# jiwoon-ahn/irn

Measured on AMD Instinct MI355X. Metric: images/sec for CAM+random-walk label gen, VOC12 512^2 (random-walk label generation stage), higher is better.
Workload: dtype f32

## Files before the change

irn_amd/csrc/label.hip:

```cpp
#include "kernels.hpp"

#pragma clang fp contract(off)

namespace irn {

struct LabelJob {
    const float *rw;
    const int64_t *keys;
    uint8_t *labels;
    int32_t *argmax;
    float *rw_up;
    unsigned *max_slot;
    int c, h, w, oh, ow;
    const uint8_t *gt;
};

namespace {

__device__ __forceinline__ unsigned enc_ordered(float f) {
    const unsigned b = __float_as_uint(f);
    return (b & 0x80000000u) ? ~b : (b | 0x80000000u);
}
__device__ __forceinline__ float dec_ordered(unsigned u) {
    return __uint_as_float((u & 0x80000000u) ? (u & 0x7fffffffu) : ~u);
}

struct Taps {
    int i0, i1;
    float l0, l1;
};

__device__ __forceinline__ Taps taps_x4(int dst, int n_in) {
    float src = ((float)dst + 0.5f) * 0.25f;
    src = src - 0.5f;
    src = src < 0.f ? 0.f : src;
    Taps t;
    t.i0 = min((int)src, n_in - 1);
    t.i1 = min(t.i0 + 1, n_in - 1);
    t.l1 = src - (float)t.i0;
    t.l0 = 1.0f - t.l1;
    return t;
}

__device__ __forceinline__ float bilerp(const float *__restrict__ plane, int w, const Taps &ty, const Taps &tx) {
    const float v00 = plane[ty.i0 * w + tx.i0], v01 = plane[ty.i0 * w + tx.i1];
    const float v10 = plane[ty.i1 * w + tx.i0], v11 = plane[ty.i1 * w + tx.i1];
    const float p01 = v01 * tx.l1, p11 = v11 * tx.l1;
    const float top = __builtin_fmaf(v00, tx.l0, p01);
    const float bot = __builtin_fmaf(v10, tx.l0, p11);
    const float pb = ty.l1 * bot;
    return __builtin_fmaf(ty.l0, top, pb);
}

__device__ __forceinline__ int cell_lo(int k) { return k == 0 ? 0 : 4 * k + 2; }

template <int PASS>
__global__ __launch_bounds__(256) void upsample_max_kernel(const LabelJob *__restrict__ jobs) {
    const LabelJob J = jobs[blockIdx.y];
    const unsigned plane_px = (unsigned)(J.h * J.w), cells = (unsigned)J.c * plane_px;
    const float lower = PASS == 2 ? dec_ordered(*J.max_slot) : 0.f;
    float m = -INFINITY;
    for (unsigned i = blockIdx.x * 256 + threadIdx.x; i < cells; i += gridDim.x * 256) {
        const int c = (int)(i / plane_px);
        const int r = (int)(i - (unsigned)c * plane_px);
        const int k = (int)((unsigned)r / (unsigned)J.w), l = r - k * J.w;
        const int y0 = cell_lo(k), x0 = cell_lo(l);
        if (y0 >= J.oh || x0 >= J.ow) continue;
        const float *plane = J.rw + (long)c * J.h * J.w;
        if (PASS == 1) {
            m = fmaxf(m, bilerp(plane, J.w, taps_x4(y0, J.h), taps_x4(x0, J.w)));
        } else {
            const int k1 = min(k + 1, J.h - 1), l1 = min(l + 1, J.w - 1);
            const float u = fmaxf(fmaxf(plane[k * J.w + l], plane[k * J.w + l1]), fmaxf(plane[k1 * J.w + l], plane[k1 * J.w + l1]));
            if (u + fabsf(u) * 1e-6f + 1e-37f < lower) continue;
            const int y1 = min(k == J.h - 1 ? 4 * J.h - 1 : 4 * k + 5, J.oh - 1);
            const int x1 = min(l == J.w - 1 ? 4 * J.w - 1 : 4 * l + 5, J.ow - 1);
            for (int oy = y0; oy <= y1; ++oy) {
                const Taps ty = taps_x4(oy, J.h);
                for (int ox = x0; ox <= x1; ++ox) m = fmaxf(m, bilerp(plane, J.w, ty, taps_x4(ox, J.w)));
            }
        }
    }
    for (int s = 32; s > 0; s >>= 1) m = fmaxf(m, __shfl_xor(m, s));
    __shared__ float wmax[4];
    if ((threadIdx.x & 63) == 0) wmax[threadIdx.x >> 6] = m;
    __syncthreads();
    if (threadIdx.x == 0) {
        m = fmaxf(fmaxf(wmax[0], wmax[1]), fmaxf(wmax[2], wmax[3]));
        if (m > -INFINITY) atomicMax(J.max_slot, enc_ordered(m));
    }
}

__device__ __forceinline__ float bilerp_vals(float v00, float v01, float v10, float v11, const Taps &ty, const Taps &tx) {
    const float p01 = v01 * tx.l1, p11 = v11 * tx.l1;
    const float top = __builtin_fmaf(v00, tx.l0, p01);
    const float bot = __builtin_fmaf(v10, tx.l0, p11);
    const float pb = ty.l1 * bot;
    return __builtin_fmaf(ty.l0, top, pb);
}

__global__ __launch_bounds__(256) void label_argmax_kernel(const LabelJob *__restrict__ jobs, float bg) {
    const LabelJob J = jobs[blockIdx.y];
    const unsigned gw = (unsigned)(J.ow + 3) >> 2, groups = gw * (unsigned)J.oh;
    const unsigned npx = (unsigned)J.oh * (unsigned)J.ow;
    const float gmax = dec_ordered(*J.max_slot);
    for (unsigned g = blockIdx.x * 256 + threadIdx.x; g < groups; g += gridDim.x * 256) {
        const int oy = (int)(g / gw), ox = (int)(g - (unsigned)oy * gw) * 4;
        const int nq = min(4, J.ow - ox);
        const Taps ty = taps_x4(oy, J.h);
        Taps tx[4];
#pragma unroll
        for (int q = 0; q < 4; ++q) tx[q] = taps_x4(min(ox + q, J.ow - 1), J.w);
        float best[4] = {bg, bg, bg, bg};
        int idx[4] = {0, 0, 0, 0};
        const unsigned o = (unsigned)oy * (unsigned)J.ow + (unsigned)ox;
        for (int c = 0; c < J.c; ++c) {
            const float *r0 = J.rw + (long)c * J.h * J.w + ty.i0 * J.w, *r1 = J.rw + (long)c * J.h * J.w + ty.i1 * J.w;
            const float a00 = r0[tx[0].i0], a01 = r0[tx[0].i1], a10 = r1[tx[0].i0], a11 = r1[tx[0].i1];
            const float b00 = r0[tx[2].i0], b01 = r0[tx[2].i1], b10 = r1[tx[2].i0], b11 = r1[tx[2].i1];
            float v[4];
            v[0] = bilerp_vals(a00, a01, a10, a11, ty, tx[0]) / gmax;
            v[1] = bilerp_vals(a00, a01, a10, a11, ty, tx[1]) / gmax;
            v[2] = bilerp_vals(b00, b01, b10, b11, ty, tx[2]) / gmax;
            v[3] = bilerp_vals(b00, b01, b10, b11, ty, tx[3]) / gmax;
            if (J.rw_up) {
                float *dst = J.rw_up + (long)c * npx + o;
                if (nq == 4 && ((uintptr_t)dst & 15) == 0) *reinterpret_cast<float4 *>(dst) = make_float4(v[0], v[1], v[2], v[3]);
                else
                    for (int q = 0; q < nq; ++q) dst[q] = v[q];
            }
#pragma unroll
            for (int q = 0; q < 4; ++q)
                if (v[q] > best[q] || (v[q] != v[q] && best[q] == best[q])) {
                    best[q] = v[q];
                    idx[q] = c + 1;
                }
        }
        if (J.argmax) {
            int32_t *dst = J.argmax + o;
            if (nq == 4 && ((uintptr_t)dst & 15) == 0) *reinterpret_cast<int4 *>(dst) = make_int4(idx[0], idx[1], idx[2], idx[3]);
            else
                for (int q = 0; q < nq; ++q) dst[q] = idx[q];
        }
        if (J.labels) {
            uint8_t lab[4];
#pragma unroll
            for (int q = 0; q < 4; ++q) lab[q] = idx[q] == 0 ? (uint8_t)0 : (uint8_t)(J.keys[idx[q] - 1] + 1);
            uint8_t *dst = J.labels + o;
            if (nq == 4 && ((uintptr_t)dst & 3) == 0)
                *reinterpret_cast<uint32_t *>(dst) = (uint32_t)lab[0] | ((uint32_t)lab[1] << 8) | ((uint32_t)lab[2] << 16) | ((uint32_t)lab[3] << 24);
            else
                for (int q = 0; q < nq; ++q) dst[q] = lab[q];
        }
    }
}

constexpr int kSweepGroups = 4;
constexpr int kSweepChunk = 256 * kSweepGroups;
constexpr int kSweepCap = 15360;
constexpr int kSweepRows = IRN_EVAL_CLASSES + 1;
constexpr int kSweepMaxC = IRN_EVAL_CLASSES - 1;
constexpr uint32_t kSweepSkip = 0xffffffffu;

__global__ __launch_bounds__(256) void label_sweep_kernel(const LabelJob *__restrict__ jobs, const float *__restrict__ thres,
                                                          int t, int cap, int64_t *__restrict__ hist, int64_t *__restrict__ bad) {
    extern __shared__ __attribute__((aligned(16))) uint32_t sweep_lds[];
    uint32_t *bins = sweep_lds;
    float *th = reinterpret_cast<float *>(sweep_lds + cap);
    int *col = reinterpret_cast<int *>(th + IRN_EVAL_MAX_THRES);
    uint32_t *nbad = reinterpret_cast<uint32_t *>(col + kSweepMaxC);
    const LabelJob J = jobs[blockIdx.y];
    const int tid = threadIdx.x;
    if (tid == 0) *nbad = 0;
    for (int i = tid; i < t; i += 256) th[i] = thres[i];
    if (tid < J.c) {
        const int64_t key = J.keys[tid];
        col[tid] = (key >= 0 && key < kSweepMaxC) ? (int)key + 1 : -1;
    }
    __syncthreads();
    uint32_t local_bad = 0;
    if (blockIdx.x == 0 && blockIdx.y == 0)
        for (int i = tid; i < t; i += 256)
            if (th[i] != th[i] || (i > 0 && !(th[i - 1] <= th[i]))) ++local_bad;

    const unsigned gw = (unsigned)(J.ow + 3) >> 2, groups = gw * (unsigned)J.oh;
    const unsigned chunks = (groups + kSweepChunk - 1) / kSweepChunk;
    const uint32_t nbins = (uint32_t)(t + 1) * kSweepRows * (uint32_t)J.c;
    const float gmax = dec_ordered(*J.max_slot);
    for (unsigned chunk = blockIdx.x; chunk < chunks; chunk += gridDim.x) {
        uint32_t bin[4 * kSweepGroups];
#pragma unroll
        for (int i = 0; i < kSweepGroups; ++i) {
#pragma unroll
            for (int q = 0; q < 4; ++q) bin[4 * i + q] = kSweepSkip;
            const unsigned g = chunk * kSweepChunk + (unsigned)i * 256 + (unsigned)tid;
            if (g >= groups) continue;
            const int oy = (int)(g / gw), ox = (int)(g - (unsigned)oy * gw) * 4;
            const int nq = min(4, J.ow - ox);
            const Taps ty = taps_x4(oy, J.h);
            Taps tx[4];
#pragma unroll
            for (int q = 0; q < 4; ++q) tx[q] = taps_x4(min(ox + q, J.ow - 1), J.w);
            float m[4] = {0.f, 0.f, 0.f, 0.f};
            int cs[4] = {0, 0, 0, 0}, nanc[4] = {-1, -1, -1, -1};
            for (int c = 0; c < J.c; ++c) {
                const float *r0 = J.rw + (long)c * J.h * J.w + ty.i0 * J.w, *r1 = J.rw + (long)c * J.h * J.w + ty.i1 * J.w;
                const float a00 = r0[tx[0].i0], a01 = r0[tx[0].i1], a10 = r1[tx[0].i0], a11 = r1[tx[0].i1];
                const float b00 = r0[tx[2].i0], b01 = r0[tx[2].i1], b10 = r1[tx[2].i0], b11 = r1[tx[2].i1];
                float v[4];
                v[0] = bilerp_vals(a00, a01, a10, a11, ty, tx[0]) / gmax;
                v[1] = bilerp_vals(a00, a01, a10, a11, ty, tx[1]) / gmax;
                v[2] = bilerp_vals(b00, b01, b10, b11, ty, tx[2]) / gmax;
                v[3] = bilerp_vals(b00, b01, b10, b11, ty, tx[3]) / gmax;
#pragma unroll
                for (int q = 0; q < 4; ++q) {
                    if (c == 0 || v[q] > m[q]) {
                        m[q] = v[q];
                        cs[q] = c;
                    }
                    if (v[q] != v[q] && nanc[q] < 0) nanc[q] = c;
                }
            }
            const uint8_t *gp = J.gt + ((unsigned)oy * (unsigned)J.ow + (unsigned)ox);
            uint8_t gv[4] = {0, 0, 0, 0};
            if (nq == 4 && ((uintptr_t)gp & 3) == 0) {
                const uint32_t u = *reinterpret_cast<const uint32_t *>(gp);
                gv[0] = (uint8_t)u; gv[1] = (uint8_t)(u >> 8); gv[2] = (uint8_t)(u >> 16); gv[3] = (uint8_t)(u >> 24);
            } else {
                for (int q = 0; q < nq; ++q) gv[q] = gp[q];
            }
#pragma unroll
            for (int q = 0; q < 4; ++q) {
                if (q >= nq) continue;
                const int row = gv[q] <= 20 ? (int)gv[q] : (gv[q] == 255 ? IRN_EVAL_CLASSES : -1);
                if (row < 0) {
                    ++local_bad;
                    continue;
                }
                int lo = 0, hi = t;
                while (lo < hi) {
                    const int mid = (lo + hi) >> 1;
                    if (th[mid] < m[q]) lo = mid + 1;
                    else hi = mid;
                }
                const int j = nanc[q] >= 0 ? t : lo, cq = nanc[q] >= 0 ? nanc[q] : cs[q];
                bin[4 * i + q] = ((uint32_t)j * kSweepRows + (uint32_t)row) * (uint32_t)J.c + (uint32_t)cq;
            }
        }
        for (uint32_t b0 = 0; b0 < nbins; b0 += (uint32_t)cap) {
            const uint32_t nb = min((uint32_t)cap, nbins - b0);
            for (uint32_t b = tid; b < nb; b += 256) bins[b] = 0;
            __syncthreads();
#pragma unroll
            for (int i = 0; i < 4 * kSweepGroups; ++i)
                if (bin[i] - b0 < nb) atomicAdd(&bins[bin[i] - b0], 1u);
            __syncthreads();
            for (uint32_t b = tid; b < nb; b += 256) {
                const uint32_t v = bins[b];
                if (!v) continue;
                const uint32_t id = b0 + b;
                const int c = (int)(id % (uint32_t)J.c);
                const uint32_t r = id / (uint32_t)J.c;
                const int row = (int)(r % kSweepRows), j = (int)(r / kSweepRows);
                if (col[c] < 0) {
                    local_bad += v;
                    continue;
                }
                atomicAdd(reinterpret_cast<unsigned long long *>(hist + ((size_t)row * IRN_EVAL_CLASSES + col[c]) * (t + 1) + j),
                          (unsigned long long)v);
            }
            __syncthreads();
        }
    }
    if (local_bad) atomicAdd(nbad, local_bad);
    __syncthreads();
    if (tid == 0 && *nbad) atomicAdd(reinterpret_cast<unsigned long long *>(bad), (unsigned long long)*nbad);
}

constexpr int kMaxScales = 8;
struct MergeArgs {
    const float *src[kMaxScales];
    int hs[kMaxScales], ws[kMaxScales];
    int n_scales, n_cls, k;
    const int64_t *keys;
    float *lo, *hi;
    int lh, lw, uh, uw, H, W;
    unsigned *max_slots;
};

__device__ __forceinline__ Taps taps_resize(int dst, int n_in, int n_out) {
    const float scale = (float)n_in / (float)n_out;
    float src = scale * ((float)dst + 0.5f);
    src = src - 0.5f;
    src = src < 0.f ? 0.f : src;
    Taps t;
    t.i0 = min((int)src, n_in - 1);
    t.i1 = min(t.i0 + 1, n_in - 1);
    t.l1 = src - (float)t.i0;
    t.l0 = 1.0f - t.l1;
    return t;
}

__global__ __launch_bounds__(256) void cam_merge_sum_kernel(const MergeArgs A) {
    const int kk = blockIdx.y;
    const bool is_hi = blockIdx.z == 1;
    const int oh = is_hi ? A.H : A.lh, ow = is_hi ? A.W : A.lw;
    const int th = is_hi ? A.uh : A.lh, tw = is_hi ? A.uw : A.lw;
    float *out = (is_hi ? A.hi : A.lo) + (long)kk * oh * ow;
    const int cls = (int)A.keys[kk];
    float m = -INFINITY;
    for (long o = (long)blockIdx.x * 256 + threadIdx.x; o < (long)oh * ow; o += (long)gridDim.x * 256) {
        const int oy = (int)(o / ow), ox = (int)(o - (long)oy * ow);
        float acc = 0.f;
        for (int s = 0; s < A.n_scales; ++s) {
            const Taps ty = taps_resize(oy, A.hs[s], th), tx = taps_resize(ox, A.ws[s], tw);
            acc = acc + bilerp(A.src[s] + (long)cls * A.hs[s] * A.ws[s], A.ws[s], ty, tx);
        }
        out[o] = acc;
        m = fmaxf(m, acc);
    }
    for (int s = 32; s > 0; s >>= 1) m = fmaxf(m, __shfl_xor(m, s));
    __shared__ float wmax[4];
    if ((threadIdx.x & 63) == 0) wmax[threadIdx.x >> 6] = m;
    __syncthreads();
    if (threadIdx.x == 0) {
        m = fmaxf(fmaxf(wmax[0], wmax[1]), fmaxf(wmax[2], wmax[3]));
        if (m > -INFINITY) atomicMax(A.max_slots + (is_hi ? A.k : 0) + kk, enc_ordered(m));
    }
}

__global__ __launch_bounds__(256) void cam_merge_norm_kernel(const MergeArgs A) {
    const int kk = blockIdx.y;
    const bool is_hi = blockIdx.z == 1;
    const long n = is_hi ? (long)A.H * A.W : (long)A.lh * A.lw;
    float *out = (is_hi ? A.hi : A.lo) + (long)kk * n;
    const float den = dec_ordered(A.max_slots[(is_hi ? A.k : 0) + kk]) + 1e-5f;
    for (long o = (long)blockIdx.x * 256 + threadIdx.x; o < n; o += (long)gridDim.x * 256) out[o] = out[o] / den;
}

}
}

using namespace irn;

extern "C" int irn_label_epilogue(int n_images, const float *const *rw_dev, const int32_t *c, const int32_t *h,
                                  const int32_t *w, const int32_t *out_h, const int32_t *out_w, float bg_thres,
                                  const int64_t *const *keys_dev, uint8_t *const *labels_dev,
                                  int32_t *const *argmax_dev, float *const *rw_up_dev, void *scratch_dev,
                                  void *stream_) {
    hipStream_t stream = (hipStream_t)stream_;
    if (n_images < 1 || !rw_dev || !c || !h || !w || !out_h || !out_w || !scratch_dev)
        return fail(IRN_ERR_ARG, "irn_label_epilogue: bad argument");
    std::vector<LabelJob> jobs(n_images);
    long max_px = 0, max_cells = 0;
    for (int i = 0; i < n_images; ++i) {
        LabelJob &J = jobs[i];
        if (!rw_dev[i] || c[i] < 1 || h[i] < 1 || w[i] < 1 || out_h[i] < 1 || out_w[i] < 1 ||
            out_h[i] > 4 * h[i] || out_w[i] > 4 * w[i])
            return fail(IRN_ERR_ARG, "irn_label_epilogue: image %d: bad sizes (c=%d %dx%d -> %dx%d)", i, c[i], h[i],
                        w[i], out_h[i], out_w[i]);
        J.rw = rw_dev[i];
        J.keys = keys_dev ? keys_dev[i] : nullptr;
        J.labels = labels_dev ? labels_dev[i] : nullptr;
        J.argmax = argmax_dev ? argmax_dev[i] : nullptr;
        J.rw_up = rw_up_dev ? rw_up_dev[i] : nullptr;
        if (J.labels && !J.keys)
            return fail(IRN_ERR_ARG, "irn_label_epilogue: image %d: labels requested without keys", i);
        J.max_slot = (unsigned *)scratch_dev + i;
        J.c = c[i]; J.h = h[i]; J.w = w[i]; J.oh = out_h[i]; J.ow = out_w[i];
        max_px = std::max(max_px, (long)out_h[i] * out_w[i]);
        max_cells = std::max(max_cells, (long)c[i] * h[i] * w[i]);
    }
    LabelJob *jobs_dev = nullptr;
    int rc = scratch_upload(jobs.data(), sizeof(LabelJob) * n_images, (void **)&jobs_dev, stream);
    if (rc) return rc;
    IRN_HIP_TRY(hipMemsetAsync(scratch_dev, 0, sizeof(unsigned) * n_images, stream));
    if (max_px >= (1L << 31) || max_cells >= (1L << 31)) return fail(IRN_ERR_ARG, "irn_label_epilogue: image too large (32-bit pixel indices)");
    const long per_image = std::max<long>(1, 4096 / n_images);
    const int bx = (int)std::min<long>((max_px / 4 + 255) / 256 + 1, 512);
    const int bc = (int)std::min<long>((max_cells + 255) / 256, per_image);
    hipLaunchKernelGGL(upsample_max_kernel<1>, dim3(bc, n_images), dim3(256), 0, stream, jobs_dev);
    IRN_LAUNCH_CHECK("upsample_max_kernel<1>");
    hipLaunchKernelGGL(upsample_max_kernel<2>, dim3(bc, n_images), dim3(256), 0, stream, jobs_dev);
    IRN_LAUNCH_CHECK("upsample_max_kernel<2>");
    hipLaunchKernelGGL(label_argmax_kernel, dim3(bx, n_images), dim3(256), 0, stream, jobs_dev, bg_thres);
    IRN_LAUNCH_CHECK("label_argmax_kernel");
    return scratch_release(stream);
}

extern "C" int irn_label_sweep_confusion(int n_images, const float *const *rw_dev, const int32_t *c, const int32_t *h,
                                         const int32_t *w, const int32_t *out_h, const int32_t *out_w,
                                         const int64_t *const *keys_dev, const uint8_t *const *gt_dev,
                                         const float *thres_dev, int t, int64_t *hist_dev, int64_t *bad_dev,
                                         void *scratch_dev, void *stream_) {
    hipStream_t stream = (hipStream_t)stream_;
    if (n_images < 1 || n_images > 65535 || !rw_dev || !c || !h || !w || !out_h || !out_w || !keys_dev || !gt_dev || !thres_dev ||
        !hist_dev || !bad_dev || !scratch_dev || t < 1 || t > IRN_EVAL_MAX_THRES)
        return fail(IRN_ERR_ARG, "irn_label_sweep_confusion: bad argument (n_images=%d, t=%d; 1 <= t <= %d)", n_images, t,
                    IRN_EVAL_MAX_THRES);
    std::vector<LabelJob> jobs(n_images);
    long max_px = 0, max_cells = 0;
    int max_c = 0;
    for (int i = 0; i < n_images; ++i) {
        LabelJob &J = jobs[i];
        if (!rw_dev[i] || c[i] < 1 || c[i] > kSweepMaxC || h[i] < 1 || w[i] < 1 || out_h[i] < 1 || out_w[i] < 1 ||
            out_h[i] > 4 * h[i] || out_w[i] > 4 * w[i])
            return fail(IRN_ERR_ARG, "irn_label_sweep_confusion: image %d: bad sizes (c=%d %dx%d -> %dx%d; 1 <= c <= %d)", i,
                        c[i], h[i], w[i], out_h[i], out_w[i], kSweepMaxC);
        if (!keys_dev[i] || !gt_dev[i])
            return fail(IRN_ERR_ARG, "irn_label_sweep_confusion: image %d: keys and ground truth are required", i);
        J.rw = rw_dev[i];
        J.keys = keys_dev[i];
        J.labels = nullptr;
        J.argmax = nullptr;
        J.rw_up = nullptr;
        J.gt = gt_dev[i];
        J.max_slot = (unsigned *)scratch_dev + i;
        J.c = c[i]; J.h = h[i]; J.w = w[i]; J.oh = out_h[i]; J.ow = out_w[i];
        max_px = std::max(max_px, (long)out_h[i] * out_w[i]);
        max_cells = std::max(max_cells, (long)c[i] * h[i] * w[i]);
        max_c = std::max(max_c, c[i]);
    }
    if (max_px >= (1L << 31) || max_cells >= (1L << 31))
        return fail(IRN_ERR_ARG, "irn_label_sweep_confusion: image too large (32-bit pixel indices)");
    LabelJob *jobs_dev = nullptr;
    int rc = scratch_upload(jobs.data(), sizeof(LabelJob) * n_images, (void **)&jobs_dev, stream);
    if (rc) return rc;
    IRN_HIP_TRY(hipMemsetAsync(scratch_dev, 0, sizeof(unsigned) * n_images, stream));
    const long per_image = std::max<long>(1, 4096 / n_images);
    const int bc = (int)std::min<long>((max_cells + 255) / 256, per_image);
    hipLaunchKernelGGL(upsample_max_kernel<1>, dim3(bc, n_images), dim3(256), 0, stream, jobs_dev);
    IRN_LAUNCH_CHECK("upsample_max_kernel<1>");
    hipLaunchKernelGGL(upsample_max_kernel<2>, dim3(bc, n_images), dim3(256), 0, stream, jobs_dev);
    IRN_LAUNCH_CHECK("upsample_max_kernel<2>");
    const long nbins = (long)(t + 1) * kSweepRows * max_c;
    const int cap = (int)std::min<long>((nbins + 3) / 4 * 4, kSweepCap);
    const size_t lds = sizeof(uint32_t) * cap + sizeof(float) * IRN_EVAL_MAX_THRES + sizeof(int) * kSweepMaxC + sizeof(uint32_t);
    const int bx = (int)std::min<long>(((max_px + 3) / 4 + kSweepChunk - 1) / kSweepChunk + 1, 128);
    hipLaunchKernelGGL(label_sweep_kernel, dim3(bx, n_images), dim3(256), lds, stream, jobs_dev, thres_dev, t, cap, hist_dev,
                       bad_dev);
    IRN_LAUNCH_CHECK("label_sweep_kernel");
    return scratch_release(stream);
}

extern "C" int irn_cam_merge(int n_scales, const float *const *src_dev, const int32_t *hs, const int32_t *ws, int n_classes,
                             const int64_t *keys_dev, int n_keys, int out_h, int out_w, float *cam_dev,
                             float *high_res_dev, void *scratch_dev, void *stream_) {
    hipStream_t stream = (hipStream_t)stream_;
    if (n_scales < 1 || n_scales > kMaxScales || !src_dev || !hs || !ws || n_classes < 1 || !keys_dev || n_keys < 1 ||
        out_h < 1 || out_w < 1 || !cam_dev || !high_res_dev || !scratch_dev)
        return fail(IRN_ERR_ARG, "irn_cam_merge: bad argument (1..%d scales, >= 1 key)", kMaxScales);
    MergeArgs A;
    for (int s = 0; s < n_scales; ++s) {
        if (!src_dev[s] || hs[s] < 1 || ws[s] < 1) return fail(IRN_ERR_ARG, "irn_cam_merge: scale %d: bad input", s);
        A.src[s] = src_dev[s];
        A.hs[s] = hs[s];
        A.ws[s] = ws[s];
    }
    A.n_scales = n_scales;
    A.n_cls = n_classes;
    A.k = n_keys;
    A.keys = keys_dev;
    A.lo = cam_dev;
    A.hi = high_res_dev;
    A.H = out_h;
    A.W = out_w;
    A.lh = (out_h - 1) / 4 + 1;
    A.lw = (out_w - 1) / 4 + 1;
    A.uh = ((out_h - 1) / 16 + 1) * 16;
    A.uw = ((out_w - 1) / 16 + 1) * 16;
    A.max_slots = (unsigned *)scratch_dev;
    IRN_HIP_TRY(hipMemsetAsync(scratch_dev, 0, sizeof(unsigned) * 2 * n_keys, stream));
    const int bx = (int)std::min<long>(((long)out_h * out_w + 255) / 256, 256);
    hipLaunchKernelGGL(cam_merge_sum_kernel, dim3(bx, n_keys, 2), dim3(256), 0, stream, A);
    IRN_LAUNCH_CHECK("cam_merge_sum_kernel");
    hipLaunchKernelGGL(cam_merge_norm_kernel, dim3(bx, n_keys, 2), dim3(256), 0, stream, A);
    IRN_LAUNCH_CHECK("cam_merge_norm_kernel");
    return IRN_OK;
}
```

Measured before the change: 19660.

## Fuse upsample-max passes per channel and compute argmax on 4x4 output blocks

Merges the two upsample-max passes into one kernel that runs one block per (image, channel). It computes a coarse lower bound, gathers candidate cells into LDS, and evaluates their full 6x6 windows cooperatively. The label argmax kernel now produces 4x4 output tiles from a shared 3x3 source neighbourhood with fixed x4 weights. It also swaps the per-value division by gmax for a comparison against a precomputed threshold, and falls back to the exact quotient test only when ties are challenged. This is meant to cut redundant loads, divisions and a kernel launch, but it adds complexity and floating-point equivalence logic that must match the original rounding.

```diff
diff --git a/irn_amd/csrc/label.hip b/irn_amd/csrc/label.hip
--- a/irn_amd/csrc/label.hip
+++ b/irn_amd/csrc/label.hip
@@ -1,3 +1,5 @@
+#include <cfloat>
+
 #include "kernels.hpp"
 
 #pragma clang fp contract(off)
@@ -54,41 +56,91 @@
 
 __device__ __forceinline__ int cell_lo(int k) { return k == 0 ? 0 : 4 * k + 2; }
 
-template <int PASS>
-__global__ __launch_bounds__(256) void upsample_max_kernel(const LabelJob *__restrict__ jobs) {
-    const LabelJob J = jobs[blockIdx.y];
-    const unsigned plane_px = (unsigned)(J.h * J.w), cells = (unsigned)J.c * plane_px;
-    const float lower = PASS == 2 ? dec_ordered(*J.max_slot) : 0.f;
-    float m = -INFINITY;
-    for (unsigned i = blockIdx.x * 256 + threadIdx.x; i < cells; i += gridDim.x * 256) {
-        const int c = (int)(i / plane_px);
-        const int r = (int)(i - (unsigned)c * plane_px);
-        const int k = (int)((unsigned)r / (unsigned)J.w), l = r - k * J.w;
-        const int y0 = cell_lo(k), x0 = cell_lo(l);
-        if (y0 >= J.oh || x0 >= J.ow) continue;
-        const float *plane = J.rw + (long)c * J.h * J.w;
-        if (PASS == 1) {
-            m = fmaxf(m, bilerp(plane, J.w, taps_x4(y0, J.h), taps_x4(x0, J.w)));
-        } else {
-            const int k1 = min(k + 1, J.h - 1), l1 = min(l + 1, J.w - 1);
-            const float u = fmaxf(fmaxf(plane[k * J.w + l], plane[k * J.w + l1]), fmaxf(plane[k1 * J.w + l], plane[k1 * J.w + l1]));
-            if (u + fabsf(u) * 1e-6f + 1e-37f < lower) continue;
-            const int y1 = min(k == J.h - 1 ? 4 * J.h - 1 : 4 * k + 5, J.oh - 1);
-            const int x1 = min(l == J.w - 1 ? 4 * J.w - 1 : 4 * l + 5, J.ow - 1);
-            for (int oy = y0; oy <= y1; ++oy) {
-                const Taps ty = taps_x4(oy, J.h);
-                for (int ox = x0; ox <= x1; ++ox) m = fmaxf(m, bilerp(plane, J.w, ty, taps_x4(ox, J.w)));
-            }
-        }
-    }
+constexpr int kMaxThreads = 1024;
+constexpr int kRows = 4;
+constexpr int kCand = 1024;
+
+__device__ __forceinline__ float block_max(float m, float *wmax) {
     for (int s = 32; s > 0; s >>= 1) m = fmaxf(m, __shfl_xor(m, s));
-    __shared__ float wmax[4];
     if ((threadIdx.x & 63) == 0) wmax[threadIdx.x >> 6] = m;
     __syncthreads();
-    if (threadIdx.x == 0) {
-        m = fmaxf(fmaxf(wmax[0], wmax[1]), fmaxf(wmax[2], wmax[3]));
-        if (m > -INFINITY) atomicMax(J.max_slot, enc_ordered(m));
-    }
+    m = wmax[0];
+    for (unsigned i = 1; i < (blockDim.x >> 6); ++i) m = fmaxf(m, wmax[i]);
+    __syncthreads();
+    return m;
+}
+
+__device__ __forceinline__ void eval_cell(const float *__restrict__ plane, const LabelJob &J, int k, int l, int j0, int j1, float &m, bool &nan) {
+    const int y0 = cell_lo(k), x0 = cell_lo(l);
+    const int y1 = min(k == J.h - 1 ? 4 * J.h - 1 : 4 * k + 5, J.oh - 1);
+    const int x1 = min(l == J.w - 1 ? 4 * J.w - 1 : 4 * l + 5, J.ow - 1);
+    for (int j = j0; j < j1; ++j) {
+        const int oy = y0 + j / 6, ox = x0 + j % 6;
+        if (oy > y1 || ox > x1) continue;
+        const float o = bilerp(plane, J.w, taps_x4(oy, J.h), taps_x4(ox, J.w));
+        nan |= o != o;
+        m = fmaxf(m, o);
+    }
+}
+
+__global__ __launch_bounds__(kMaxThreads) void upsample_max_kernel(const LabelJob *__restrict__ jobs) {
+    const LabelJob J = jobs[blockIdx.x];
+    if ((int)blockIdx.y >= J.c) return;
+    __shared__ float wmax[kMaxThreads / 64];
+    __shared__ unsigned cand[kCand], n_cand;
+    if (threadIdx.x == 0) n_cand = 0;
+    const float *plane = J.rw + (long)blockIdx.y * J.h * J.w;
+    const int wave = __builtin_amdgcn_readfirstlane(threadIdx.x >> 6), lane = threadIdx.x & 63, n_waves = blockDim.x >> 6;
+    const int rows = min(J.h, max(1, (J.oh + 1) / 4)), cols = min(J.w, max(1, (J.ow + 1) / 4));
+    float m = -INFINITY;
+    for (int kb = wave; kb < rows; kb += kRows * n_waves) {
+        Taps ty[kRows];
+#pragma unroll
+        for (int i = 0; i < kRows; ++i) ty[i] = taps_x4(cell_lo(min(kb + i * n_waves, rows - 1)), J.h);
+        for (int l = lane; l < cols; l += 64) {
+            const Taps tx = taps_x4(cell_lo(l), J.w);
+            float v[kRows];
+#pragma unroll
+            for (int i = 0; i < kRows; ++i) v[i] = bilerp(plane, J.w, ty[i], tx);
+#pragma unroll
+            for (int i = 0; i < kRows; ++i)
+                if (kb + i * n_waves < rows) m = fmaxf(m, v[i]);
+        }
+    }
+    const float lower = block_max(m, wmax);
+    bool nan = false;
+    for (int kb = wave; kb < rows; kb += kRows * n_waves) {
+        for (int l = lane; l < cols; l += 64) {
+            const int l1 = min(l + 1, J.w - 1);
+            float v00[kRows], v01[kRows], v10[kRows], v11[kRows];
+#pragma unroll
+            for (int i = 0; i < kRows; ++i) {
+                const int k = min(kb + i * n_waves, rows - 1), k1 = min(k + 1, J.h - 1);
+                v00[i] = plane[k * J.w + l], v01[i] = plane[k * J.w + l1], v10[i] = plane[k1 * J.w + l], v11[i] = plane[k1 * J.w + l1];
+            }
+#pragma unroll
+            for (int i = 0; i < kRows; ++i) {
+                const int k = kb + i * n_waves;
+                if (k >= rows) break;
+                const float z = ((v00[i] - v00[i]) + (v01[i] - v01[i])) + ((v10[i] - v10[i]) + (v11[i] - v11[i]));
+                const float u = fmaxf(fmaxf(v00[i], v01[i]), fmaxf(v10[i], v11[i]));
+                if (z == 0.f && u + fabsf(u) * 1e-6f + 1e-37f < lower) continue;
+                const unsigned slot = atomicAdd(&n_cand, 1u);
+                if (slot < kCand) cand[slot] = (unsigned)(k * J.w + l);
+                else eval_cell(plane, J, k, l, 0, 36, m, nan);
+            }
+        }
+    }
+    __syncthreads();
+    const unsigned n_items = min(n_cand, (unsigned)kCand) * 36u;
+    for (unsigned item = threadIdx.x; item < n_items; item += blockDim.x) {
+        const unsigned cell = cand[item / 36u];
+        const int k = (int)(cell / (unsigned)J.w), l = (int)cell - k * J.w;
+        eval_cell(plane, J, k, l, (int)(item % 36u), (int)(item % 36u) + 1, m, nan);
+    }
+    if (nan) atomicMax(J.max_slot, 0xffffffffu);
+    m = block_max(m, wmax);
+    if (threadIdx.x == 0 && m > -INFINITY) atomicMax(J.max_slot, enc_ordered(m));
 }
 
 __device__ __forceinline__ float bilerp_vals(float v00, float v01, float v10, float v11, const Taps &ty, const Taps &tx) {
@@ -99,11 +151,9 @@
     return __builtin_fmaf(ty.l0, top, pb);
 }
 
-__global__ __launch_bounds__(256) void label_argmax_kernel(const LabelJob *__restrict__ jobs, float bg) {
-    const LabelJob J = jobs[blockIdx.y];
+__device__ __forceinline__ void argmax_quotients(const LabelJob &J, float gmax, float bg) {
     const unsigned gw = (unsigned)(J.ow + 3) >> 2, groups = gw * (unsigned)J.oh;
     const unsigned npx = (unsigned)J.oh * (unsigned)J.ow;
-    const float gmax = dec_ordered(*J.max_slot);
     for (unsigned g = blockIdx.x * 256 + threadIdx.x; g < groups; g += gridDim.x * 256) {
         const int oy = (int)(g / gw), ox = (int)(g - (unsigned)oy * gw) * 4;
         const int nq = min(4, J.ow - ox);
@@ -155,6 +205,148 @@
     }
 }
 
+constexpr int kLut = 256;
+
+__device__ __forceinline__ float float_step(float f, int d) { return dec_ordered(enc_ordered(f) + (unsigned)d); }
+
+__device__ __forceinline__ bool bg_threshold(float g, float bg, float *T) {
+    const float t0 = fminf(fmaxf(bg * g, -FLT_MAX), FLT_MAX);
+    const int d = (int)(threadIdx.x & 15) - 4;
+    const unsigned le = (unsigned)__ballot(float_step(t0, d) / g <= bg) & 0x3ffu;
+    const int ones = __builtin_ctz(~le);
+    *T = float_step(t0, ones - 5);
+    return g > 0.f && g < INFINITY && fabsf(bg) < INFINITY && ones >= 1 && ones <= 9 && le == (1u << ones) - 1u;
+}
+
+struct BlockTaps {
+    int lo, mid, hi;
+    float l0[4], l1[4];
+};
+
+__device__ __forceinline__ BlockTaps block_taps(int a, int n) {
+    BlockTaps t;
+    t.lo = max(a - 1, 0);
+    t.hi = min(a + 1, n - 1);
+    t.mid = a == 0 ? t.hi : a;
+    t.l1[0] = a == 0 ? 0.f : 0.625f;
+    t.l1[1] = a == 0 ? 0.f : 0.875f;
+    t.l1[2] = 0.125f;
+    t.l1[3] = 0.375f;
+#pragma unroll
+    for (int q = 0; q < 4; ++q) t.l0[q] = 1.0f - t.l1[q];
+    return t;
+}
+
+__global__ __launch_bounds__(256) void label_argmax_kernel(const LabelJob *__restrict__ jobs, float bg) {
+    const LabelJob J = jobs[blockIdx.y];
+    __shared__ uint8_t lut[kLut];
+    const float gmax = dec_ordered(*J.max_slot);
+    float T;
+    const bool ordered = bg_threshold(gmax, bg, &T) && !J.rw_up && (!J.labels || J.c < kLut);
+    if (!ordered) {
+        argmax_quotients(J, gmax, bg);
+        return;
+    }
+    if (J.labels) {
+        if (threadIdx.x == 0) lut[0] = 0;
+        for (int i = threadIdx.x; i < J.c; i += 256) lut[i + 1] = (uint8_t)(J.keys[i] + 1);
+        __syncthreads();
+    }
+    const unsigned bw = (unsigned)(J.ow + 3) >> 2, blocks = bw * ((unsigned)(J.oh + 3) >> 2);
+    const long plane_px = (long)J.h * J.w;
+    const bool wide = (J.ow & 3) == 0 && ((uintptr_t)J.labels & 3) == 0 && ((uintptr_t)J.argmax & 15) == 0;
+    for (unsigned g = blockIdx.x * 256 + threadIdx.x; g < blocks; g += gridDim.x * 256) {
+        const int a = (int)(g / bw), b = (int)(g - (unsigned)a * bw);
+        const int oy = 4 * a, ox = 4 * b;
+        const int nr = min(4, J.oh - oy), nq = min(4, J.ow - ox);
+        const BlockTaps ty = block_taps(a, J.h), tx = block_taps(b, J.w);
+        const int r0 = ty.lo * J.w, r1 = ty.mid * J.w, r2 = ty.hi * J.w;
+        const bool row0 = a == 0, col0 = b == 0;
+        float best[4][4];
+        int idx[4][4];
+        for (int c = 0; c < J.c; ++c) {
+            const float *p = J.rw + c * plane_px;
+            const float v[3][3] = {{p[r0 + tx.lo], p[r0 + tx.mid], p[r0 + tx.hi]},
+                                   {p[r1 + tx.lo], p[r1 + tx.mid], p[r1 + tx.hi]},
+                                   {p[r2 + tx.lo], p[r2 + tx.mid], p[r2 + tx.hi]}};
+            float H[3][4];
+#pragma unroll
+            for (int r = 0; r < 3; ++r) {
+                const float left = col0 ? v[r][0] : v[r][1];
+                const float p0 = v[r][1] * tx.l1[0], p1 = v[r][1] * tx.l1[1], p2 = v[r][2] * tx.l1[2], p3 = v[r][2] * tx.l1[3];
+                H[r][0] = __builtin_fmaf(v[r][0], tx.l0[0], p0);
+                H[r][1] = __builtin_fmaf(v[r][0], tx.l0[1], p1);
+                H[r][2] = __builtin_fmaf(left, tx.l0[2], p2);
+                H[r][3] = __builtin_fmaf(left, tx.l0[3], p3);
+            }
+            float val[4][4];
+#pragma unroll
+            for (int q = 0; q < 4; ++q) {
+                const float top23 = row0 ? H[0][q] : H[1][q];
+                const float b0 = ty.l1[0] * H[1][q], b1 = ty.l1[1] * H[1][q], b2 = ty.l1[2] * H[2][q], b3 = ty.l1[3] * H[2][q];
+                val[0][q] = __builtin_fmaf(ty.l0[0], H[0][q], b0);
+                val[1][q] = __builtin_fmaf(ty.l0[1], H[0][q], b1);
+                val[2][q] = __builtin_fmaf(ty.l0[2], top23, b2);
+                val[3][q] = __builtin_fmaf(ty.l0[3], top23, b3);
+            }
+            if (c == 0) {
+#pragma unroll
+                for (int r = 0; r < 4; ++r)
+#pragma unroll
+                    for (int q = 0; q < 4; ++q) {
+                        const bool wins = val[r][q] > T;
+                        best[r][q] = wins ? val[r][q] : T;
+                        idx[r][q] = wins ? 1 : 0;
+                    }
+                continue;
+            }
+            bool challenged = false;
+#pragma unroll
+            for (int r = 0; r < 4; ++r)
+#pragma unroll
+                for (int q = 0; q < 4; ++q) {
+                    const bool larger = val[r][q] > best[r][q], held = idx[r][q] != 0;
+                    challenged |= larger && held;
+                    if (larger && !held) {
+                        best[r][q] = val[r][q];
+                        idx[r][q] = c + 1;
+                    }
+                }
+            if (challenged) {
+#pragma unroll
+                for (int r = 0; r < 4; ++r)
+#pragma unroll
+                    for (int q = 0; q < 4; ++q)
+                        if (val[r][q] > best[r][q] && idx[r][q] != c + 1 && val[r][q] / gmax > best[r][q] / gmax) {
+                            best[r][q] = val[r][q];
+                            idx[r][q] = c + 1;
+                        }
+            }
+        }
+        const unsigned o = (unsigned)oy * (unsigned)J.ow + (unsigned)ox;
+        if (wide && nr == 4 && nq == 4) {
+#pragma unroll
+            for (int r = 0; r < 4; ++r) {
+                if (J.argmax) *reinterpret_cast<int4 *>(J.argmax + o + r * J.ow) = make_int4(idx[r][0], idx[r][1], idx[r][2], idx[r][3]);
+                if (J.labels)
+                    *reinterpret_cast<uint32_t *>(J.labels + o + r * J.ow) =
+                        (uint32_t)lut[idx[r][0]] | ((uint32_t)lut[idx[r][1]] << 8) | ((uint32_t)lut[idx[r][2]] << 16) | ((uint32_t)lut[idx[r][3]] << 24);
+            }
+            continue;
+        }
+#pragma unroll
+        for (int r = 0; r < 4; ++r) {
+            if (r >= nr) break;
+#pragma unroll
+            for (int q = 0; q < 4; ++q) {
+                if (q >= nq) break;
+                if (J.argmax) J.argmax[o + r * J.ow + q] = idx[r][q];
+                if (J.labels) J.labels[o + r * J.ow + q] = lut[idx[r][q]];
+            }
+        }
+    }
+}
+
 constexpr int kSweepGroups = 4;
 constexpr int kSweepChunk = 256 * kSweepGroups;
 constexpr int kSweepCap = 15360;
@@ -343,6 +535,18 @@
 
 using namespace irn;
 
+namespace {
+
+int launch_upsample_max(const LabelJob *jobs_dev, int n_images, int max_c, long max_plane, hipStream_t stream) {
+    if (max_c > 65535) return fail(IRN_ERR_ARG, "label epilogue: %d channels (at most 65535)", max_c);
+    const int threads = max_plane >= 4 * kMaxThreads ? kMaxThreads : 256;
+    hipLaunchKernelGGL(upsample_max_kernel, dim3(n_images, max_c), dim3(threads), 0, stream, jobs_dev);
+    IRN_LAUNCH_CHECK("upsample_max_kernel");
+    return IRN_OK;
+}
+
+}
+
 extern "C" int irn_label_epilogue(int n_images, const float *const *rw_dev, const int32_t *c, const int32_t *h,
                                   const int32_t *w, const int32_t *out_h, const int32_t *out_w, float bg_thres,
                                   const int64_t *const *keys_dev, uint8_t *const *labels_dev,
@@ -352,7 +556,9 @@
     if (n_images < 1 || !rw_dev || !c || !h || !w || !out_h || !out_w || !scratch_dev)
         return fail(IRN_ERR_ARG, "irn_label_epilogue: bad argument");
     std::vector<LabelJob> jobs(n_images);
-    long max_px = 0, max_cells = 0;
+    long max_px = 0, max_cells = 0, max_plane = 0, max_blocks = 0;
+    int max_c = 0;
+    bool any_rw_up = false;
     for (int i = 0; i < n_images; ++i) {
         LabelJob &J = jobs[i];
         if (!rw_dev[i] || c[i] < 1 || h[i] < 1 || w[i] < 1 || out_h[i] < 1 || out_w[i] < 1 ||
@@ -370,19 +576,19 @@
         J.c = c[i]; J.h = h[i]; J.w = w[i]; J.oh = out_h[i]; J.ow = out_w[i];
         max_px = std::max(max_px, (long)out_h[i] * out_w[i]);
         max_cells = std::max(max_cells, (long)c[i] * h[i] * w[i]);
+        max_plane = std::max(max_plane, (long)h[i] * w[i]);
+        max_blocks = std::max(max_blocks, (long)((out_h[i] + 3) / 4) * ((out_w[i] + 3) / 4));
+        max_c = std::max(max_c, c[i]);
+        any_rw_up = any_rw_up || J.rw_up;
     }
     LabelJob *jobs_dev = nullptr;
     int rc = scratch_upload(jobs.data(), sizeof(LabelJob) * n_images, (void **)&jobs_dev, stream);
     if (rc) return rc;
     IRN_HIP_TRY(hipMemsetAsync(scratch_dev, 0, sizeof(unsigned) * n_images, stream));
     if (max_px >= (1L << 31) || max_cells >= (1L << 31)) return fail(IRN_ERR_ARG, "irn_label_epilogue: image too large (32-bit pixel indices)");
-    const long per_image = std::max<long>(1, 4096 / n_images);
-    const int bx = (int)std::min<long>((max_px / 4 + 255) / 256 + 1, 512);
-    const int bc = (int)std::min<long>((max_cells + 255) / 256, per_image);
-    hipLaunchKernelGGL(upsample_max_kernel<1>, dim3(bc, n_images), dim3(256), 0, stream, jobs_dev);
-    IRN_LAUNCH_CHECK("upsample_max_kernel<1>");
-    hipLaunchKernelGGL(upsample_max_kernel<2>, dim3(bc, n_images), dim3(256), 0, stream, jobs_dev);
-    IRN_LAUNCH_CHECK("upsample_max_kernel<2>");
+    const int bx = (int)std::min<long>(any_rw_up ? (max_px / 4 + 255) / 256 + 1 : (max_blocks + 255) / 256, 512);
+    rc = launch_upsample_max(jobs_dev, n_images, max_c, max_plane, stream);
+    if (rc) return rc;
     hipLaunchKernelGGL(label_argmax_kernel, dim3(bx, n_images), dim3(256), 0, stream, jobs_dev, bg_thres);
     IRN_LAUNCH_CHECK("label_argmax_kernel");
     return scratch_release(stream);
@@ -399,7 +605,7 @@
         return fail(IRN_ERR_ARG, "irn_label_sweep_confusion: bad argument (n_images=%d, t=%d; 1 <= t <= %d)", n_images, t,
                     IRN_EVAL_MAX_THRES);
     std::vector<LabelJob> jobs(n_images);
-    long max_px = 0, max_cells = 0;
+    long max_px = 0, max_cells = 0, max_plane = 0;
     int max_c = 0;
     for (int i = 0; i < n_images; ++i) {
         LabelJob &J = jobs[i];
@@ -419,6 +625,7 @@
         J.c = c[i]; J.h = h[i]; J.w = w[i]; J.oh = out_h[i]; J.ow = out_w[i];
         max_px = std::max(max_px, (long)out_h[i] * out_w[i]);
         max_cells = std::max(max_cells, (long)c[i] * h[i] * w[i]);
+        max_plane = std::max(max_plane, (long)h[i] * w[i]);
         max_c = std::max(max_c, c[i]);
     }
     if (max_px >= (1L << 31) || max_cells >= (1L << 31))
@@ -427,12 +634,8 @@
     int rc = scratch_upload(jobs.data(), sizeof(LabelJob) * n_images, (void **)&jobs_dev, stream);
     if (rc) return rc;
     IRN_HIP_TRY(hipMemsetAsync(scratch_dev, 0, sizeof(unsigned) * n_images, stream));
-    const long per_image = std::max<long>(1, 4096 / n_images);
-    const int bc = (int)std::min<long>((max_cells + 255) / 256, per_image);
-    hipLaunchKernelGGL(upsample_max_kernel<1>, dim3(bc, n_images), dim3(256), 0, stream, jobs_dev);
-    IRN_LAUNCH_CHECK("upsample_max_kernel<1>");
-    hipLaunchKernelGGL(upsample_max_kernel<2>, dim3(bc, n_images), dim3(256), 0, stream, jobs_dev);
-    IRN_LAUNCH_CHECK("upsample_max_kernel<2>");
+    rc = launch_upsample_max(jobs_dev, n_images, max_c, max_plane, stream);
+    if (rc) return rc;
     const long nbins = (long)(t + 1) * kSweepRows * max_c;
     const int cap = (int)std::min<long>((nbins + 3) / 4 * 4, kSweepCap);
     const size_t lds = sizeof(uint32_t) * cap + sizeof(float) * IRN_EVAL_MAX_THRES + sizeof(int) * kSweepMaxC + sizeof(uint32_t);
```

New measurement: 19810, median of 6. About the same (+0.7%).
